# mpc001/auto_avsr

Hardware: AMD Instinct MI355X
Metric: video-frames/sec/node (25fps 88x88, max-frames=1600), E2E training step (fwd+bwd+clip+AdamW) (higher is better)
Workload: dtype f16 activations x f16x2 weights (atrunk3, atrunk4, decoder, encoder, trunk3, trunk4) + split-bf16 (everything else) forward / bf16 backward

## Files before the change

auto_avsr_amd/csrc/prims.h:

```cpp
#pragma once

extern "C" void avsr_note_launch(int err);
extern "C" int avsr_take_launch_error(void);
#ifdef AVSR_EMU
#include "hip_emu.h"
#define AVSR_LAUNCH(kern, grid, block, smem, stream, ...) \
    emu::launch((grid), (block), (smem), [=]() { kern(__VA_ARGS__); })
#define AVSR_DYN_SMEM(name) char* name = emu::dyn_smem()
#else
#include <hip/hip_runtime.h>
#define AVSR_LAUNCH(kern, grid, block, smem, stream, ...)                          \
    do {                                                                           \
        (void)hipGetLastError();                                                   \
        hipLaunchKernelGGL(kern, (grid), (block), (smem), (stream), __VA_ARGS__);  \
        avsr_note_launch((int)hipGetLastError());                                  \
    } while (0)
#define AVSR_DYN_SMEM(name) extern __shared__ __attribute__((aligned(16))) char name[]
#endif

#include <stdint.h>

#define AVSR_DEV __device__ __forceinline__
#define AVSR_WAVE 64

typedef uint16_t bf16_t;
typedef short bf16x8 __attribute__((ext_vector_type(8)));
typedef short bf16x4 __attribute__((ext_vector_type(4)));
typedef float f32x4 __attribute__((ext_vector_type(4)));
typedef float f32x16 __attribute__((ext_vector_type(16)));

AVSR_DEV float bf2f(bf16_t h) {
    uint32_t u = ((uint32_t)h) << 16;
    return __builtin_bit_cast(float, u);
}
AVSR_DEV bf16_t f2bf(float f) {
#ifndef AVSR_EMU
    return __builtin_bit_cast(bf16_t, (__bf16)f);
#endif
    uint32_t u = __builtin_bit_cast(uint32_t, f);
    if ((u & 0x7fffffffu) > 0x7f800000u) return (bf16_t)((u >> 16) | 0x40);
    u += 0x7fffu + ((u >> 16) & 1u);
    return (bf16_t)(u >> 16);
}

typedef _Float16 f16_t;
typedef _Float16 f16x8 __attribute__((ext_vector_type(8)));
typedef _Float16 f16x4 __attribute__((ext_vector_type(4)));
AVSR_DEV float h2f(f16_t h) { return (float)h; }
AVSR_DEV f16_t f2h(float f) {
#ifdef AVSR_EMU
    f = f > 65504.f ? 65504.f : (f < -65504.f ? -65504.f : f);
#else
    f = __builtin_amdgcn_fmed3f(f, -65504.f, 65504.f);
#endif
    return (f16_t)f;
}
AVSR_DEV short f2h_bits(float f) { return __builtin_bit_cast(short, f2h(f)); }
#define AVSR_H16_LO_SCALE 2048.0f
AVSR_DEV f16_t f2h_lo(float w) { return f2h((w - h2f(f2h(w))) * AVSR_H16_LO_SCALE); }

template <class T> struct Elem;
template <> struct Elem<float> {
    static AVSR_DEV float ld(const float* p) { return *p; }
    static AVSR_DEV void st(float* p, float v) { *p = v; }
};
template <> struct Elem<bf16_t> {
    static AVSR_DEV float ld(const bf16_t* p) { return bf2f(*p); }
    static AVSR_DEV void st(bf16_t* p, float v) { *p = f2bf(v); }
};
template <> struct Elem<f16_t> {
    static AVSR_DEV float ld(const f16_t* p) { return h2f(*p); }
    static AVSR_DEV void st(f16_t* p, float v) { *p = f2h(v); }
};

AVSR_DEV void load8(const bf16_t* p, float* out) {
    bf16x8 v = *reinterpret_cast<const bf16x8*>(p);
#pragma unroll
    for (int i = 0; i < 8; i++) out[i] = bf2f((bf16_t)v[i]);
}
AVSR_DEV void load8(const f16_t* p, float* out) {
    f16x8 v = *reinterpret_cast<const f16x8*>(p);
#pragma unroll
    for (int i = 0; i < 8; i++) out[i] = (float)v[i];
}
AVSR_DEV void load8(const float* p, float* out) {
    f32x4 a = *reinterpret_cast<const f32x4*>(p);
    f32x4 b = *reinterpret_cast<const f32x4*>(p + 4);
#pragma unroll
    for (int i = 0; i < 4; i++) {
        out[i] = a[i];
        out[i + 4] = b[i];
    }
}
AVSR_DEV void store8(bf16_t* p, const float* v) {
    bf16x8 o;
#pragma unroll
    for (int i = 0; i < 8; i++) o[i] = (short)f2bf(v[i]);
    *reinterpret_cast<bf16x8*>(p) = o;
}
AVSR_DEV void store8(f16_t* p, const float* v) {
    f16x8 o;
#pragma unroll
    for (int i = 0; i < 8; i++) o[i] = f2h(v[i]);
    *reinterpret_cast<f16x8*>(p) = o;
}
AVSR_DEV void store8_lo(f16_t* p, const float* v) {
    float l[8];
#pragma unroll
    for (int i = 0; i < 8; i++) l[i] = (v[i] - h2f(f2h(v[i]))) * AVSR_H16_LO_SCALE;
    store8(p, l);
}
AVSR_DEV void store8(float* p, const float* v) {
    f32x4 a, b;
#pragma unroll
    for (int i = 0; i < 4; i++) {
        a[i] = v[i];
        b[i] = v[i + 4];
    }
    *reinterpret_cast<f32x4*>(p) = a;
    *reinterpret_cast<f32x4*>(p + 4) = b;
}

AVSR_DEV void glds16(const void* gptr, void* lds_wave_base) {
#ifdef AVSR_EMU
    memcpy(reinterpret_cast<char*>(lds_wave_base) + 16 * emu::lane_id(), gptr, 16);
#else
    __builtin_amdgcn_global_load_lds((const __attribute__((address_space(1))) void*)gptr,
                                     (__attribute__((address_space(3))) void*)lds_wave_base, 16, 0, 0);
#endif
}
AVSR_DEV void block_barrier_raw() {
#ifdef AVSR_EMU
    emu::sync_threads();
#else
    __builtin_amdgcn_s_barrier();
#endif
}
AVSR_DEV int wave_id() {
#ifdef AVSR_EMU
    return (int)(threadIdx.x >> 6);
#else
    return __builtin_amdgcn_readfirstlane((int)(threadIdx.x >> 6));
#endif
}
AVSR_DEV void sched_fence() {
#ifndef AVSR_EMU
    __builtin_amdgcn_sched_barrier(0);
#endif
}
template <int N> AVSR_DEV void wait_vmcnt() {
#ifndef AVSR_EMU
    asm volatile("s_waitcnt vmcnt(%0)" ::"n"(N) : "memory");
#endif
}

AVSR_DEV bf16x4 lds_tr16(const bf16_t* p) {
#ifdef AVSR_EMU
    bf16x4 mine = *reinterpret_cast<const bf16x4*>(p);
    size_t stride;
    const unsigned char* all = emu::wave_gather(&mine, sizeof(mine), &stride);
    const int l = emu::lane_id(), i = l & 15, g = l >> 4;
    bf16x4 out;
    for (int j = 0; j < 4; j++) {
        bf16x4 src;
        memcpy(&src, all + (size_t)(16 * g + 4 * j + (i >> 2)) * stride, sizeof(src));
        out[j] = src[i & 3];
    }
    return out;
#else
    return __builtin_amdgcn_ds_read_tr16_b64_v4i16((__attribute__((address_space(3))) bf16x4*)p);
#endif
}

AVSR_DEV bf16x4 lds_tr16_async(const bf16_t* p) {
#ifdef AVSR_EMU
    return lds_tr16(p);
#else
    const uint32_t addr = (uint32_t)(uintptr_t)(const __attribute__((address_space(3))) bf16_t*)p;
    bf16x4 v;
    asm volatile("ds_read_b64_tr_b16 %0, %1" : "=v"(v) : "v"(addr));
    return v;
#endif
}
typedef int i32x4 __attribute__((ext_vector_type(4)));
typedef int i32x2 __attribute__((ext_vector_type(2)));
AVSR_DEV i32x4 lds_read16_async(const void* p) {
#ifdef AVSR_EMU
    i32x4 v;
    memcpy(&v, p, 16);
    return v;
#else
    const uint32_t addr = (uint32_t)(uintptr_t)(const __attribute__((address_space(3))) char*)p;
    i32x4 v;
    asm volatile("ds_read_b128 %0, %1" : "=v"(v) : "v"(addr));
    return v;
#endif
}
AVSR_DEV i32x2 lds_read8_async(const void* p) {
#ifdef AVSR_EMU
    i32x2 v;
    memcpy(&v, p, 8);
    return v;
#else
    const uint32_t addr = (uint32_t)(uintptr_t)(const __attribute__((address_space(3))) char*)p;
    i32x2 v;
    asm volatile("ds_read_b64 %0, %1" : "=v"(v) : "v"(addr));
    return v;
#endif
}
template <int N> AVSR_DEV void lds_wait() {
#ifndef AVSR_EMU
    asm volatile("s_waitcnt lgkmcnt(%0)" ::"n"(N));
#endif
}
template <class T> AVSR_DEV void lds_tie(T& v) {
#ifndef AVSR_EMU
    asm volatile("" : "+v"(v));
#endif
}

AVSR_DEV float avsr_exp(float x) {
#ifdef AVSR_EMU
    return expf(x);
#else
    return __expf(x);
#endif
}
AVSR_DEV float avsr_sigmoid(float x) {
#ifdef AVSR_EMU
    return 1.0f / (1.0f + avsr_exp(-x));
#else
    return __builtin_amdgcn_rcpf(1.0f + avsr_exp(-x));
#endif
}
AVSR_DEV float avsr_silu(float x) { return x * avsr_sigmoid(x); }

AVSR_DEV float wave_up1(float x, float fill) {
#ifdef AVSR_EMU
    const float v = __shfl_up(x, 1);
    return emu::lane_id() == 0 ? fill : v;
#else
    return __int_as_float(__builtin_amdgcn_update_dpp(__float_as_int(fill), __float_as_int(x), 0x138, 0xf, 0xf, false));
#endif
}
AVSR_DEV float wave_down1(float x, float fill) {
#ifdef AVSR_EMU
    const float v = __shfl_down(x, 1);
    return emu::lane_id() == 63 ? fill : v;
#else
    return __int_as_float(__builtin_amdgcn_update_dpp(__float_as_int(fill), __float_as_int(x), 0x130, 0xf, 0xf, false));
#endif
}

AVSR_DEV float wave_sum(float v) {
#pragma unroll
    for (int m = 32; m >= 1; m >>= 1) v += __shfl_xor(v, m);
    return v;
}
AVSR_DEV float wave_max(float v) {
#pragma unroll
    for (int m = 32; m >= 1; m >>= 1) v = fmaxf(v, __shfl_xor(v, m));
    return v;
}

AVSR_DEV f32x16 mfma32(bf16x8 a, bf16x8 b, f32x16 c) {
#ifdef AVSR_EMU
    struct P { bf16x8 a, b; } mine{a, b};
    size_t stride;
    const unsigned char* all = emu::wave_gather(&mine, sizeof(P), &stride);
    const int l = emu::lane_id();
    const int j = l & 31;
    for (int r = 0; r < 16; r++) {
        const int i = (r & 3) + 8 * (r >> 2) + 4 * (l >> 5);
        float acc = c[r];
        for (int kb = 0; kb < 2; kb++) {
            P pa, pb;
            memcpy(&pa, all + (size_t)(i + 32 * kb) * stride, sizeof(P));
            memcpy(&pb, all + (size_t)(j + 32 * kb) * stride, sizeof(P));
            for (int e = 0; e < 8; e++) acc += bf2f((bf16_t)pa.a[e]) * bf2f((bf16_t)pb.b[e]);
        }
        c[r] = acc;
    }
    return c;
#else
    typedef __bf16 v8bf __attribute__((ext_vector_type(8)));
    return __builtin_amdgcn_mfma_f32_32x32x16_bf16(__builtin_bit_cast(v8bf, a),
                                                   __builtin_bit_cast(v8bf, b), c, 0, 0, 0);
#endif
}
AVSR_DEV f32x16 mfma32_vgpr(bf16x8 a, bf16x8 b, f32x16 c) {
#ifdef AVSR_EMU
    return mfma32(a, b, c);
#else
    asm volatile("v_mfma_f32_32x32x16_bf16 %0, %1, %2, %0" : "+v"(c) : "v"(a), "v"(b));
    return c;
#endif
}
AVSR_DEV f32x4 mfma16(bf16x8 a, bf16x8 b, f32x4 c) {
#ifdef AVSR_EMU
    struct P { bf16x8 a, b; } mine{a, b};
    size_t stride;
    const unsigned char* all = emu::wave_gather(&mine, sizeof(P), &stride);
    const int l = emu::lane_id();
    const int j = l & 15;
    for (int r = 0; r < 4; r++) {
        const int i = 4 * (l >> 4) + r;
        float acc = c[r];
        for (int kb = 0; kb < 4; kb++) {
            P pa, pb;
            memcpy(&pa, all + (size_t)(i + 16 * kb) * stride, sizeof(P));
            memcpy(&pb, all + (size_t)(j + 16 * kb) * stride, sizeof(P));
            for (int e = 0; e < 8; e++) acc += bf2f((bf16_t)pa.a[e]) * bf2f((bf16_t)pb.b[e]);
        }
        c[r] = acc;
    }
    return c;
#else
    typedef __bf16 v8bf __attribute__((ext_vector_type(8)));
    return __builtin_amdgcn_mfma_f32_16x16x32_bf16(__builtin_bit_cast(v8bf, a),
                                                   __builtin_bit_cast(v8bf, b), c, 0, 0, 0);
#endif
}

template <int FMT> AVSR_DEV float raw16_to_f32(short bits) {
    return FMT == 1 ? (float)__builtin_bit_cast(f16_t, bits) : bf2f((bf16_t)bits);
}
template <int FMT> AVSR_DEV short f32_to_raw16(float v) { return FMT == 1 ? f2h_bits(v) : (short)f2bf(v); }
template <int FMT> AVSR_DEV f32x16 mfma32x(bf16x8 a, bf16x8 b, f32x16 c) {
    if (FMT == 0) return mfma32(a, b, c);
#ifdef AVSR_EMU
    struct P { bf16x8 a, b; } mine{a, b};
    size_t stride;
    const unsigned char* all = emu::wave_gather(&mine, sizeof(P), &stride);
    const int l = emu::lane_id();
    const int j = l & 31;
    for (int r = 0; r < 16; r++) {
        const int i = (r & 3) + 8 * (r >> 2) + 4 * (l >> 5);
        float acc = c[r];
        for (int kb = 0; kb < 2; kb++) {
            P pa, pb;
            memcpy(&pa, all + (size_t)(i + 32 * kb) * stride, sizeof(P));
            memcpy(&pb, all + (size_t)(j + 32 * kb) * stride, sizeof(P));
            for (int e = 0; e < 8; e++) acc += raw16_to_f32<1>(pa.a[e]) * raw16_to_f32<1>(pb.b[e]);
        }
        c[r] = acc;
    }
    return c;
#else
    return __builtin_amdgcn_mfma_f32_32x32x16_f16(__builtin_bit_cast(f16x8, a), __builtin_bit_cast(f16x8, b), c, 0, 0, 0);
#endif
}
template <int FMT> AVSR_DEV f32x4 mfma16x(bf16x8 a, bf16x8 b, f32x4 c) {
    if (FMT == 0) return mfma16(a, b, c);
#ifdef AVSR_EMU
    struct P { bf16x8 a, b; } mine{a, b};
    size_t stride;
    const unsigned char* all = emu::wave_gather(&mine, sizeof(P), &stride);
    const int l = emu::lane_id();
    const int j = l & 15;
    for (int r = 0; r < 4; r++) {
        const int i = 4 * (l >> 4) + r;
        float acc = c[r];
        for (int kb = 0; kb < 4; kb++) {
            P pa, pb;
            memcpy(&pa, all + (size_t)(i + 16 * kb) * stride, sizeof(P));
            memcpy(&pb, all + (size_t)(j + 16 * kb) * stride, sizeof(P));
            for (int e = 0; e < 8; e++) acc += raw16_to_f32<1>(pa.a[e]) * raw16_to_f32<1>(pb.b[e]);
        }
        c[r] = acc;
    }
    return c;
#else
    return __builtin_amdgcn_mfma_f32_16x16x32_f16(__builtin_bit_cast(f16x8, a), __builtin_bit_cast(f16x8, b), c, 0, 0, 0);
#endif
}

template <int NS> struct Frag { bf16x8 p[NS]; };

template <int NS>
AVSR_DEV f32x16 mma32(const Frag<NS>& a, const Frag<NS>& b, f32x16 c) {
    if (NS == 2) {
        c = mfma32(a.p[NS - 1], b.p[0], c);
        c = mfma32(a.p[0], b.p[NS - 1], c);
    }
    return mfma32(a.p[0], b.p[0], c);
}
template <int NS>
AVSR_DEV f32x4 mma16(const Frag<NS>& a, const Frag<NS>& b, f32x4 c) {
    if (NS == 2) {
        c = mfma16(a.p[NS - 1], b.p[0], c);
        c = mfma16(a.p[0], b.p[NS - 1], c);
    }
    return mfma16(a.p[0], b.p[0], c);
}

template <int NS> AVSR_DEV void split_bf16(float x, bf16_t* out) {
    bf16_t h = f2bf(x);
    out[0] = h;
    if (NS == 2) out[NS - 1] = f2bf(x - bf2f(h));
}

struct sp8_t { float raw; };
AVSR_DEV void load8(const sp8_t* p, float* out) {
    const bf16x8 hi = *reinterpret_cast<const bf16x8*>(p);
    const bf16x8 lo = *(reinterpret_cast<const bf16x8*>(p) + 1);
#pragma unroll
    for (int i = 0; i < 8; i++) out[i] = bf2f((bf16_t)hi[i]) + bf2f((bf16_t)lo[i]);
}
AVSR_DEV void store8(sp8_t* p, const float* v) {
    bf16x8 hi, lo;
#pragma unroll
    for (int i = 0; i < 8; i++) {
        bf16_t pl[2];
        split_bf16<2>(v[i], pl);
        hi[i] = (short)pl[0];
        lo[i] = (short)pl[1];
    }
    *reinterpret_cast<bf16x8*>(p) = hi;
    *(reinterpret_cast<bf16x8*>(p) + 1) = lo;
}
template <> struct Elem<sp8_t> {
    static AVSR_DEV float ld(const sp8_t*) { return 0.f; }
    static AVSR_DEV void st(sp8_t*, float) {}
};

AVSR_DEV uint32_t avsr_hash_key(uint64_t seed) {
    uint64_t z = seed + 0x9E3779B97F4A7C15ull;
    z = (z ^ (z >> 30)) * 0xBF58476D1CE4E5B9ull;
    z = (z ^ (z >> 27)) * 0x94D049BB133111EBull;
    z = z ^ (z >> 31);
    return (uint32_t)(z >> 32);
}
AVSR_DEV uint32_t avsr_mix32(uint32_t x) {
    x ^= x >> 16;
    x *= 0x7feb352du;
    x ^= x >> 15;
    x *= 0x846ca68bu;
    x ^= x >> 16;
    return x;
}
AVSR_DEV uint32_t avsr_hash(uint64_t seed, uint64_t idx) {
    uint32_t x = avsr_mix32((uint32_t)idx ^ avsr_hash_key(seed));
    const uint32_t hi = (uint32_t)(idx >> 32);
    if (hi) x = avsr_mix32(x + hi * 0x9E3779B1u);
    return x;
}
AVSR_DEV float dropout_scale(uint64_t seed, uint64_t idx, float p, float inv_keep) {
    if (p <= 0.f) return 1.f;
    const float u = (float)(avsr_hash(seed, idx) >> 8) * (1.0f / 16777216.0f);
    return u < p ? 0.f : inv_keep;
}

extern int avsr_tune_knobs[32];
inline bool avsr_det() { return avsr_tune_knobs[23] != 0; }
int avsr_colsum_det(const void* src, int dtype, long ld, long rows, int cols, float* out, hipStream_t stream);
int avsr_rowsum_det_bf16(const void* src, long ld, long rows, long cols, float* out, hipStream_t stream);
extern "C" void avsr_set_error(const char* msg);
extern "C" void avsr_set_error2(const char* where, const char* what);
#define AVSR_CHECK_LAUNCH(name)                                                   \
    do {                                                                          \
        int e__ = avsr_take_launch_error();                                       \
        if (e__ != 0) {                                                           \
            avsr_set_error2(name, hipGetErrorString((hipError_t)e__));            \
            return 2;                                                             \
        }                                                                         \
    } while (0)
#define AVSR_REQUIRE(cond, msg)         \
    do {                                \
        if (!(cond)) {                  \
            avsr_set_error(msg);        \
            return 1;                   \
        }                               \
    } while (0)
```

auto_avsr_amd/csrc/stem.hip:

```cpp
#include "prims.h"
#include "avsr_hip.h"

namespace {

constexpr int KT = 5, KH = 7, KW = 7, ROWS = KT * KH;
constexpr int KP = 288;
constexpr int CO = 64;
constexpr int LP = 104;

template <int NS>
__global__ void stem_weight_kernel(const float* __restrict__ w, bf16_t* __restrict__ wp) {
    const int i = blockIdx.x * 256 + threadIdx.x;
    if (i >= CO * KP) return;
    const int co = i / KP, k = i % KP, r = k >> 3, j = k & 7;
    bf16_t pl[NS];
    split_bf16<NS>((r < ROWS && j >= 1) ? w[(co * ROWS + r) * KW + j - 1] : 0.f, pl);
#pragma unroll
    for (int q = 0; q < NS; q++) wp[q * CO * KP + i] = pl[q];
}

constexpr int PATCH_V = 4;
template <int NS = 1>
AVSR_DEV void patch_init(bf16_t* patch, int W) {
    for (int i = threadIdx.x; i < 36 * LP; i += 256) {
        const int r = i / LP, c = i - r * LP;
        if (r == 35 || c < 4 || c >= 4 + W)
#pragma unroll
            for (int q = 0; q < NS; q++) patch[q * 36 * LP + i] = 0;
    }
}
AVSR_DEV void patch_load(f32x4 (&q)[PATCH_V], const float* __restrict__ x, long row, int OH, int T, int H, int W) {
    const int n = (int)(row / OH), oh = (int)(row - (long)n * OH);
    const int b = n / T, t = n - b * T;
    const int nv = W >> 2;
#pragma unroll
    for (int j = 0; j < PATCH_V; j++) {
        const int i = threadIdx.x + 256 * j;
        q[j] = f32x4{0.f, 0.f, 0.f, 0.f};
        if (i < ROWS * nv) {
            const int r = i / nv, v = i - r * nv;
            const int kt = r / KH, kh = r - kt * KH;
            const int tt = t + kt - 2, ih = 2 * oh + kh - 3;
            if (tt >= 0 && tt < T && ih >= 0 && ih < H)
                q[j] = *reinterpret_cast<const f32x4*>(x + (((long)b * T + tt) * H + ih) * W + v * 4);
        }
    }
}
template <int NS = 1>
AVSR_DEV void patch_store(bf16_t* patch, const f32x4 (&q)[PATCH_V], int W) {
    const int nv = W >> 2;
#pragma unroll
    for (int j = 0; j < PATCH_V; j++) {
        const int i = threadIdx.x + 256 * j;
        if (i < ROWS * nv) {
            const int r = i / nv, v = i - r * nv;
            bf16x4 o[NS];
#pragma unroll
            for (int e = 0; e < 4; e++) {
                bf16_t pl[NS];
                split_bf16<NS>(q[j][e], pl);
#pragma unroll
                for (int s = 0; s < NS; s++) o[s][e] = (short)pl[s];
            }
#pragma unroll
            for (int s = 0; s < NS; s++)
                *reinterpret_cast<bf16x4*>(patch + s * 36 * LP + r * LP + 4 + v * 4) = o[s];
        }
    }
}

AVSR_DEV bf16x8 patch_frag(const bf16_t* patch, int r, int ow) {
    const uint32_t* p = reinterpret_cast<const uint32_t*>(patch + r * LP + 2 * ow);
    bf16x8 f;
#pragma unroll
    for (int e = 0; e < 4; e++) {
        const uint32_t u = p[e];
        f[2 * e] = (short)(u & 0xffff);
        f[2 * e + 1] = (short)(u >> 16);
    }
    return f;
}

constexpr int FWD_ROWS = 8;
constexpr int OP = 72;

template <int NS, class TO>
__global__ __launch_bounds__(256) void stem_fwd_kernel(const float* __restrict__ x, const bf16_t* __restrict__ wp,
                                                       TO* __restrict__ y, int T, int H, int W, int OH, int OW,
                                                       long total_rows, bf16_t* __restrict__ y2 = nullptr,
                                                       float* __restrict__ stats_part = nullptr) {
    constexpr int OPT = sizeof(TO) == 2 ? OP : 68;
    __shared__ __attribute__((aligned(16))) bf16_t patch[NS * 36 * LP];
    __shared__ __attribute__((aligned(16))) TO orow[64 * OPT];
    const int lane = threadIdx.x & 63, w = threadIdx.x >> 6;
    const int quad = lane >> 4, lc = lane & 15;
    Frag<NS> fb[9];
#pragma unroll
    for (int ks = 0; ks < 9; ks++)
#pragma unroll
        for (int q = 0; q < NS; q++)
            fb[ks].p[q] = *reinterpret_cast<const bf16x8*>(wp + q * CO * KP + (16 * w + lc) * KP + ks * 32 + 8 * quad);
    const int ntile = (OW + 15) / 16;
    const long row_end = min(total_rows, ((long)blockIdx.x + 1) * FWD_ROWS);
    patch_init<NS>(patch, W);
    f32x4 q[PATCH_V];
    patch_load(q, x, (long)blockIdx.x * FWD_ROWS, OH, T, H, W);
    f32x4 st1 = f32x4{0.f, 0.f, 0.f, 0.f}, st2 = f32x4{0.f, 0.f, 0.f, 0.f};
    for (long row = (long)blockIdx.x * FWD_ROWS; row < row_end; row++) {
        __syncthreads();
        patch_store<NS>(patch, q, W);
        if (row + 1 < row_end) patch_load(q, x, row + 1, OH, T, H, W);
        __syncthreads();
        for (int mt = 0; mt < ntile; mt++) {
            const int ow = min(mt * 16 + lc, OW - 1);
            f32x4 acc = f32x4{0.f, 0.f, 0.f, 0.f};
#pragma unroll
            for (int ks = 0; ks < 9; ks++) {
                Frag<NS> fx;
#pragma unroll
                for (int s = 0; s < NS; s++) fx.p[s] = patch_frag(patch + s * 36 * LP, ks * 4 + quad, ow);
                acc = mma16<NS>(fb[ks], fx, acc);
            }
            TO* o = orow + (mt * 16 + lc) * OPT + 16 * w + 4 * quad;
            if (sizeof(TO) == 2) {
                *reinterpret_cast<bf16x4*>(o) = bf16x4{(short)f2bf(acc[0]), (short)f2bf(acc[1]), (short)f2bf(acc[2]), (short)f2bf(acc[3])};
            } else {
                *reinterpret_cast<f32x4*>(o) = acc;
            }
        }
        __syncthreads();
        TO* dst = y + (row * OW) * CO;
        constexpr int EPC = 16 / sizeof(TO), CPP = CO / EPC;
        for (int i = threadIdx.x; i < OW * CPP; i += 256) {
            const int pix = i / CPP, c = (i % CPP) * EPC;
            const f32x4 v = *reinterpret_cast<const f32x4*>(orow + pix * OPT + c);
            *reinterpret_cast<f32x4*>(dst + pix * CO + c) = v;
            if (sizeof(TO) == 4 && stats_part) {
#pragma unroll
                for (int e = 0; e < 4; e++) {
                    st1[e] += v[e];
                    st2[e] += v[e] * v[e];
                }
            }
            if (sizeof(TO) == 4 && y2)
                *reinterpret_cast<bf16x4*>(y2 + (row * OW + pix) * CO + c) =
                    bf16x4{(short)f2bf(v[0]), (short)f2bf(v[1]), (short)f2bf(v[2]), (short)f2bf(v[3])};
        }
    }
    if (sizeof(TO) == 4 && stats_part) {
        __syncthreads();
        float* red = reinterpret_cast<float*>(orow);
        const int grp = threadIdx.x >> 4, c = (threadIdx.x & 15) * 4;
#pragma unroll
        for (int e = 0; e < 4; e++) {
            red[(grp * 2 + 0) * CO + c + e] = st1[e];
            red[(grp * 2 + 1) * CO + c + e] = st2[e];
        }
        __syncthreads();
        if (threadIdx.x < 2 * CO) {
            float v = 0.f;
#pragma unroll
            for (int g2 = 0; g2 < 16; g2++) v += red[g2 * 2 * CO + threadIdx.x];
            stats_part[(size_t)blockIdx.x * 2 * CO + threadIdx.x] = v;
        }
    }
}

constexpr int EP = 56;
constexpr int EO_ARR = 36 * EP;
constexpr int DYP = 64;

AVSR_DEV void eo_load(float (&v)[28], const float* __restrict__ x, long row, int OH, int T, int H, int W) {
    const int tid = threadIdx.x;
    if (tid >= ROWS * 6) return;
    const int n = (int)(row / OH), oh = (int)(row - (long)n * OH);
    const int b = n / T, t = n - b * T;
    const int r = tid / 6, g = tid - r * 6;
    const int kt = r / KH, kh = r - kt * KH;
    const int tt = t + kt - 2, ih = 2 * oh + kh - 3;
    const bool row_ok = tt >= 0 && tt < T && ih >= 0 && ih < H;
    const float* src = x + (((long)b * T + tt) * H + ih) * W;
#pragma unroll
    for (int q = 0; q < 7; q++) {
        const int c = 16 * g - 4 + 4 * q;
        f32x4 f = f32x4{0.f, 0.f, 0.f, 0.f};
        if (row_ok && c >= 0 && c + 3 < W) f = *reinterpret_cast<const f32x4*>(src + c);
        else if (row_ok)
#pragma unroll
            for (int e = 0; e < 4; e++) f[e] = (c + e >= 0 && c + e < W) ? src[c + e] : 0.f;
#pragma unroll
        for (int e = 0; e < 4; e++) v[4 * q + e] = f[e];
    }
}
AVSR_DEV void eo_store(bf16_t* eo, const float (&v)[28]) {
    const int tid = threadIdx.x;
    if (tid >= ROWS * 6) return;
    const int r = tid / 6, g = tid - r * 6;
#pragma unroll
    for (int par = 0; par < 2; par++)
#pragma unroll
        for (int sh = 0; sh < 4; sh++) {
            bf16x8 o;
#pragma unroll
            for (int m = 0; m < 8; m++) o[m] = (short)f2bf(v[1 + 2 * (m + sh) + par]);
            *reinterpret_cast<bf16x8*>(eo + (par * 4 + sh) * EO_ARR + r * EP + 8 * g) = o;
        }
}

__global__ __launch_bounds__(256) void stem_wgrad_kernel(const bf16_t* __restrict__ dy, const float* __restrict__ x,
                                                         float* __restrict__ partial, int T, int H, int W, int OH, int OW,
                                                         long total_rows) {
    __shared__ __attribute__((aligned(16))) bf16_t eo[8 * EO_ARR];
    __shared__ __attribute__((aligned(16))) bf16_t dyt[64 * DYP];
    const int lane = threadIdx.x & 63, w = threadIdx.x >> 6;
    const int quad = lane >> 4, lc = lane & 15;
    f32x4 acc[5][4];
#pragma unroll
    for (int j = 0; j < 5; j++)
#pragma unroll
        for (int m = 0; m < 4; m++) acc[j][m] = f32x4{0.f, 0.f, 0.f, 0.f};
    for (int i = threadIdx.x; i < 64 * DYP / 8; i += 256) reinterpret_cast<bf16x8*>(dyt)[i] = bf16x8{0, 0, 0, 0, 0, 0, 0, 0};
    for (int i = threadIdx.x; i < 8 * EP / 8; i += 256) {
        const int arr = i / (EP / 8), c8 = (i - arr * (EP / 8)) * 8;
        *reinterpret_cast<bf16x8*>(eo + arr * EO_ARR + 35 * EP + c8) = bf16x8{0, 0, 0, 0, 0, 0, 0, 0};
    }
    for (int i = threadIdx.x; i < 8 * 36; i += 256)
        *reinterpret_cast<bf16x8*>(eo + (i / 36) * EO_ARR + (i % 36) * EP + 48) = bf16x8{0, 0, 0, 0, 0, 0, 0, 0};
    int a_off[5];
#pragma unroll
    for (int j = 0; j < 5; j++) {
        const int kq = 16 * min(w + 4 * j, 17) + lc, r = kq >> 3, kw = kq & 7;
        a_off[j] = ((kw & 1) * 4 + (kw >> 1)) * EO_ARR + r * EP + 8 * quad;
    }
    const int b_row = 8 * quad + (lc >> 2), b_col = 4 * (lc & 3);
    float xv[28];
    bf16x8 dv[2];
    auto dy_load = [&](long row) {
#pragma unroll
        for (int j = 0; j < 2; j++) {
            const int i = threadIdx.x + 256 * j;
            dv[j] = bf16x8{0, 0, 0, 0, 0, 0, 0, 0};
            if (i < OW * 8) dv[j] = *reinterpret_cast<const bf16x8*>(dy + (row * OW + (i >> 3)) * CO + (i & 7) * 8);
        }
    };
    if ((long)blockIdx.x < total_rows) {
        eo_load(xv, x, blockIdx.x, OH, T, H, W);
        dy_load(blockIdx.x);
    }
    for (long row = blockIdx.x; row < total_rows; row += gridDim.x) {
        __syncthreads();
        eo_store(eo, xv);
#pragma unroll
        for (int j = 0; j < 2; j++) {
            const int i = threadIdx.x + 256 * j;
            if (i < OW * 8) *reinterpret_cast<bf16x8*>(dyt + (i >> 3) * DYP + (i & 7) * 8) = dv[j];
        }
        if (row + gridDim.x < total_rows) {
            eo_load(xv, x, row + gridDim.x, OH, T, H, W);
            dy_load(row + gridDim.x);
        }
        __syncthreads();
#pragma unroll
        for (int ks = 0; ks < 2; ks++) {
            bf16x8 fbm[4];
#pragma unroll
            for (int m = 0; m < 4; m++) {
                const bf16_t* p0 = dyt + (ks * 32 + b_row) * DYP + 16 * m + b_col;
                const bf16x4 lo = lds_tr16(p0), hi = lds_tr16(p0 + 4 * DYP);
                fbm[m] = bf16x8{lo[0], lo[1], lo[2], lo[3], hi[0], hi[1], hi[2], hi[3]};
            }
#pragma unroll
            for (int j = 0; j < 5; j++) {
                if (w + 4 * j >= 18) continue;
                const bf16x8 fa = *reinterpret_cast<const bf16x8*>(eo + a_off[j] + ks * 32);
#pragma unroll
                for (int m = 0; m < 4; m++) acc[j][m] = mfma16(fa, fbm[m], acc[j][m]);
            }
        }
    }
    float* out = partial + (long)blockIdx.x * KP * CO;
#pragma unroll
    for (int j = 0; j < 5; j++) {
        const int nt = w + 4 * j;
        if (nt >= 18) continue;
#pragma unroll
        for (int m = 0; m < 4; m++)
#pragma unroll
            for (int r = 0; r < 4; r++) out[(16 * nt + 4 * quad + r) * CO + 16 * m + lc] = acc[j][m][r];
    }
}

__global__ __launch_bounds__(1024) void stem_wgrad_reduce_kernel(const float* __restrict__ partial, int G,
                                                                 float* __restrict__ dw) {
    __shared__ float part[16][64];
    const int tx = threadIdx.x & 63, tz = threadIdx.x >> 6;
    const int i = blockIdx.x * 64 + tx;
    float s = 0.f;
    if (i < KP * CO)
        for (int g = tz; g < G; g += 16) s += partial[(long)g * KP * CO + i];
    part[tz][tx] = s;
    __syncthreads();
    if (tz != 0 || i >= KP * CO) return;
#pragma unroll
    for (int q = 1; q < 16; q++) s += part[q][tx];
    const int kq = i / CO, co = i - kq * CO, r = kq >> 3, kw = kq & 7;
    if (r < ROWS && kw < KW) dw[(co * ROWS + r) * KW + kw] = s;
}

}

constexpr int WG_MAX = 1024;
extern "C" int64_t avsr_stem357_workspace_bytes(void) { return (int64_t)WG_MAX * KP * CO * 4 + (int64_t)2 * CO * KP * 2; }

extern "C" int avsr_stem357_fwd(const float* x, const float* w, void* y, void* workspace, int B, int T, int H, int W,
                                hipStream_t stream) {
    AVSR_REQUIRE(W % 4 == 0 && W <= 96 && H >= 1, "stem357: W must be a multiple of 4 and <= 96");
    static_assert(ROWS * 24 <= PATCH_V * 256, "patch prefetch registers");
    if (B <= 0 || T <= 0) return 0;
    const int OH = (H + 6 - KH) / 2 + 1, OW = (W + 6 - KW) / 2 + 1;
    bf16_t* wp = reinterpret_cast<bf16_t*>(reinterpret_cast<char*>(workspace) + (size_t)WG_MAX * KP * CO * 4);
    AVSR_LAUNCH(stem_weight_kernel<1>, dim3((CO * KP + 255) / 256), dim3(256), 0, stream, w, wp);
    const long rows = (long)B * T * OH;
    AVSR_REQUIRE(OW <= 64, "stem357: at most 64 output columns");
    AVSR_LAUNCH((stem_fwd_kernel<1, bf16_t>), dim3((unsigned)((rows + FWD_ROWS - 1) / FWD_ROWS)), dim3(256), 0, stream, x,
                (const bf16_t*)wp, (bf16_t*)y, T, H, W, OH, OW, rows);
    AVSR_CHECK_LAUNCH("stem357_fwd");
    return 0;
}

static int stem357_fwd_f32s_impl(const float* x, const float* w, float* y, void* y2, void* workspace, int B, int T, int H, int W,
                                 float* stats_part, int stats_rows, hipStream_t stream) {
    AVSR_REQUIRE(W % 4 == 0 && W <= 96 && H >= 1, "stem357: W must be a multiple of 4 and <= 96");
    if (B <= 0 || T <= 0) return 0;
    const int OH = (H + 6 - KH) / 2 + 1, OW = (W + 6 - KW) / 2 + 1;
    bf16_t* wp = reinterpret_cast<bf16_t*>(reinterpret_cast<char*>(workspace) + (size_t)WG_MAX * KP * CO * 4);
    AVSR_LAUNCH(stem_weight_kernel<2>, dim3((CO * KP + 255) / 256), dim3(256), 0, stream, w, wp);
    const long rows = (long)B * T * OH;
    AVSR_REQUIRE(OW <= 64, "stem357: at most 64 output columns");
    const long blocks = (rows + FWD_ROWS - 1) / FWD_ROWS;
    AVSR_REQUIRE(stats_part == nullptr || stats_rows >= blocks, "stem357: statistics buffer too small");
    AVSR_LAUNCH((stem_fwd_kernel<2, float>), dim3((unsigned)blocks), dim3(256), 0, stream, x, (const bf16_t*)wp, y, T, H, W, OH, OW, rows,
                (bf16_t*)y2, stats_part);
    AVSR_CHECK_LAUNCH("stem357_fwd_f32s");
    return 0;
}

extern "C" int avsr_stem357_fwd_f32s(const float* x, const float* w, float* y, void* y2, void* workspace, int B, int T, int H,
                                     int W, hipStream_t stream) {
    return stem357_fwd_f32s_impl(x, w, y, y2, workspace, B, T, H, W, nullptr, 0, stream);
}
extern "C" int64_t avsr_stem357_stat_rows(int B, int T, int H) {
    const int OH = (H + 6 - KH) / 2 + 1;
    return ((int64_t)B * T * OH + FWD_ROWS - 1) / FWD_ROWS;
}
extern "C" int avsr_stem357_fwd_f32s_stats(const float* x, const float* w, float* y, void* y2, void* workspace, int B, int T, int H,
                                           int W, float* stats_part, int stats_rows, hipStream_t stream) {
    AVSR_REQUIRE(stats_part != nullptr, "stem357_fwd_f32s_stats: statistics buffer required");
    return stem357_fwd_f32s_impl(x, w, y, y2, workspace, B, T, H, W, stats_part, stats_rows, stream);
}

extern "C" int avsr_stem357_wgrad(const void* dy, const float* x, float* dw, void* workspace, int B, int T, int H, int W,
                                  hipStream_t stream) {
    AVSR_REQUIRE(W % 4 == 0 && W <= 96, "stem357: W must be a multiple of 4 and <= 96");
    if (B <= 0 || T <= 0) return 0;
    const int OH = (H + 6 - KH) / 2 + 1, OW = (W + 6 - KW) / 2 + 1;
    AVSR_REQUIRE(OW <= 64, "stem357: at most 64 output columns");
    const long rows = (long)B * T * OH;
    int gmax = avsr_tune_knobs[6] > 0 ? avsr_tune_knobs[6] : 512;
    if (gmax > WG_MAX) gmax = WG_MAX;
    const int G = (int)(rows < gmax ? rows : gmax);
    float* partial = reinterpret_cast<float*>(workspace);
    AVSR_LAUNCH(stem_wgrad_kernel, dim3(G), dim3(256), 0, stream, (const bf16_t*)dy, x, partial, T, H, W, OH, OW, rows);
    AVSR_LAUNCH(stem_wgrad_reduce_kernel, dim3((KP * CO + 63) / 64), dim3(1024), 0, stream, (const float*)partial, G, dw);
    AVSR_CHECK_LAUNCH("stem357_wgrad");
    return 0;
}
```

Before: 70110.

## Add row-group stem forward and weight-grad kernels with XCD-aware persistent scheduling

Adds new stem 3D conv forward and weight-gradient kernels that handle groups of 4 output rows per iteration. Each persistent block walks a contiguous range of groups, remapped so neighbouring ranges share an XCD, and prefetches the next group's input and dy into registers while computing the current one. The aim is to reuse the overlapping input rows across neighbouring output rows and to hide global load latency. Both kernels become the default, and the old per-row path stays behind a tune knob. The new weight-grad path also caps output width at 48 columns.

Result: faster. 70880 (median of 6 runs) (+1.1%).

```diff
diff --git a/auto_avsr_amd/csrc/prims.h b/auto_avsr_amd/csrc/prims.h
--- a/auto_avsr_amd/csrc/prims.h
+++ b/auto_avsr_amd/csrc/prims.h
@@ -146,6 +146,11 @@
 AVSR_DEV void sched_fence() {
 #ifndef AVSR_EMU
     __builtin_amdgcn_sched_barrier(0);
+#endif
+}
+template <class T> AVSR_DEV void reg_opaque(T& v) {
+#ifndef AVSR_EMU
+    asm volatile("" : "+v"(v));
 #endif
 }
 template <int N> AVSR_DEV void wait_vmcnt() {
diff --git a/auto_avsr_amd/csrc/stem.hip b/auto_avsr_amd/csrc/stem.hip
--- a/auto_avsr_amd/csrc/stem.hip
+++ b/auto_avsr_amd/csrc/stem.hip
@@ -290,6 +290,341 @@
     }
 }
 
+constexpr int WG_R = 4;
+constexpr int WG_PX = 48;
+constexpr int WG_IR = 2 * WG_R + 5;
+constexpr int WG_XR = KT * WG_IR;
+constexpr int WG_ARR = WG_XR * EP;
+constexpr int WG_XG = 7;
+constexpr int WG_XT = 2;
+constexpr int WG_DT = WG_R * WG_PX * 8 / 256;
+
+struct WgGroup {
+    int b, t, oh0;
+    long row0;
+};
+AVSR_DEV WgGroup wg_group(long grp, int GPF, int T, int OH) {
+    const int n = (int)(grp / GPF), gi = (int)(grp - (long)n * GPF);
+    WgGroup g;
+    g.b = n / T;
+    g.t = n - g.b * T;
+    g.oh0 = gi * WG_R;
+    g.row0 = (long)n * OH + g.oh0;
+    return g;
+}
+AVSR_DEV int xcd_block() {
+    const int b = blockIdx.x, total = gridDim.x, xcd = b & 7, slot = b >> 3, q = total >> 3, r = total & 7;
+    return (xcd < r ? xcd * (q + 1) : r * (q + 1) + (xcd - r) * q) + slot;
+}
+AVSR_DEV void rr_x_load(float (&v)[WG_XT][20], const float* __restrict__ x, const WgGroup& gp, int T, int H, int W) {
+#pragma unroll
+    for (int jt = 0; jt < WG_XT; jt++) {
+        const int i = min((int)threadIdx.x + 256 * jt, WG_XR * WG_XG - 1);
+        const int rs = i / WG_XG, g = i - rs * WG_XG;
+        const int kt = rs / WG_IR, li = rs - kt * WG_IR;
+        const int tt = min(max(gp.t + kt - 2, 0), T - 1), ih = min(max(2 * gp.oh0 - 3 + li, 0), H - 1);
+        const float* src = x + (((long)gp.b * T + tt) * H + ih) * W;
+#pragma unroll
+        for (int q = 0; q < 5; q++) {
+            const int c = min(max(16 * g - 4 + 4 * q, 0), W - 4);
+            const f32x4 f = *reinterpret_cast<const f32x4*>(src + c);
+#pragma unroll
+            for (int e = 0; e < 4; e++) v[jt][4 * q + e] = f[e];
+        }
+    }
+}
+AVSR_DEV void rr_x_store(bf16_t* eo, const float (&v)[WG_XT][20], const WgGroup& gp, int T, int H, int W) {
+#pragma unroll
+    for (int jt = 0; jt < WG_XT; jt++) {
+        const int i = threadIdx.x + 256 * jt;
+        if (i >= WG_XR * WG_XG) continue;
+        const int rs = i / WG_XG, g = i - rs * WG_XG;
+        const int kt = rs / WG_IR, li = rs - kt * WG_IR;
+        const int tt = gp.t + kt - 2, ih = 2 * gp.oh0 - 3 + li;
+        const bool row_ok = tt >= 0 && tt < T && ih >= 0 && ih < H;
+        bf16_t c[19];
+#pragma unroll
+        for (int j = 0; j < 19; j++) {
+            const int col = 16 * g - 4 + ((1 + j) & ~3);
+            c[j] = (row_ok && col >= 0 && col < W) ? f2bf(v[jt][1 + j]) : (bf16_t)0;
+        }
+#pragma unroll
+        for (int par = 0; par < 2; par++)
+#pragma unroll
+            for (int sh = 0; sh < 2; sh++) {
+                bf16x8 o;
+#pragma unroll
+                for (int m = 0; m < 8; m++) o[m] = (short)c[2 * (m + sh) + par];
+                *reinterpret_cast<bf16x8*>(eo + (par * 2 + sh) * WG_ARR + rs * EP + 8 * g) = o;
+            }
+    }
+}
+
+__global__ __launch_bounds__(256, 2) void stem_wgrad_rr_kernel(const bf16_t* __restrict__ dy, const float* __restrict__ x,
+                                                               float* __restrict__ partial, int T, int H, int W, int OH, int OW,
+                                                               int GPF, long groups, int per_block) {
+    __shared__ __attribute__((aligned(16))) bf16_t eo[4 * WG_ARR];
+    __shared__ __attribute__((aligned(16))) bf16_t dyt[WG_R * WG_PX * DYP];
+    const int lane = threadIdx.x & 63, w = wave_id();
+    const int quad = lane >> 4, lc = lane & 15;
+    const int lb = xcd_block();
+    const long g_begin = (long)lb * per_block, g_end = min(groups, g_begin + per_block);
+    f32x4 acc[5][4];
+#pragma unroll
+    for (int j = 0; j < 5; j++)
+#pragma unroll
+        for (int m = 0; m < 4; m++) acc[j][m] = f32x4{0.f, 0.f, 0.f, 0.f};
+    for (int i = threadIdx.x; i < WG_R * WG_PX * DYP / 8; i += 256) reinterpret_cast<bf16x8*>(dyt)[i] = bf16x8{0, 0, 0, 0, 0, 0, 0, 0};
+    int a_off[5];
+#pragma unroll
+    for (int j = 0; j < 5; j++) {
+        const int kq = 16 * min(w + 4 * j, 17) + lc, r = min(kq >> 3, ROWS - 1), kw = kq & 7;
+        const int kt = r / KH, kh = r - kt * KH;
+        a_off[j] = ((kw & 1) * 2 + ((kw >> 1) & 1)) * WG_ARR + (kt * WG_IR + kh) * EP + 2 * (kw >> 2);
+    }
+    int k_off[6];
+#pragma unroll
+    for (int ks = 0; ks < 6; ks++) {
+        const int s = 4 * ks + quad, jr = s / 6;
+        k_off[ks] = 2 * jr * EP + 8 * (s - 6 * jr);
+    }
+    const int b_row = 8 * quad + (lc >> 2), b_col = 4 * (lc & 3);
+    float xv[WG_XT][20];
+    bf16x8 dv[WG_DT];
+    auto dy_load = [&](const WgGroup& gp) {
+#pragma unroll
+        for (int jt = 0; jt < WG_DT; jt++) {
+            const int i = threadIdx.x + 256 * jt;
+            const int j = i / (WG_PX * 8), rem = i - j * (WG_PX * 8), pix = rem >> 3;
+            dv[jt] = *reinterpret_cast<const bf16x8*>(dy + ((gp.row0 + min(j, OH - 1 - gp.oh0)) * OW + min(pix, OW - 1)) * CO + (rem & 7) * 8);
+        }
+    };
+    if (g_begin < g_end) {
+        const WgGroup gp = wg_group(g_begin, GPF, T, OH);
+        rr_x_load(xv, x, gp, T, H, W);
+        dy_load(gp);
+    }
+    for (long grp = g_begin; grp < g_end; grp++) {
+        __syncthreads();
+        const WgGroup cur = wg_group(grp, GPF, T, OH);
+        const int cur_oh0 = cur.oh0;
+        rr_x_store(eo, xv, cur, T, H, W);
+#pragma unroll
+        for (int jt = 0; jt < WG_DT; jt++) {
+            const int i = threadIdx.x + 256 * jt;
+            const bool row_ok = cur_oh0 + i / (WG_PX * 8) < OH;
+            if (((i % (WG_PX * 8)) >> 3) < OW)
+                *reinterpret_cast<bf16x8*>(dyt + (i >> 3) * DYP + (i & 7) * 8) = row_ok ? dv[jt] : bf16x8{0, 0, 0, 0, 0, 0, 0, 0};
+        }
+        if (grp + 1 < g_end) {
+            const WgGroup gp = wg_group(grp + 1, GPF, T, OH);
+            rr_x_load(xv, x, gp, T, H, W);
+            dy_load(gp);
+        }
+        __syncthreads();
+#pragma unroll
+        for (int ks = 0; ks < 6; ks++) {
+            bf16x8 fbm[4];
+#pragma unroll
+            for (int m = 0; m < 4; m++) {
+                const bf16_t* p0 = dyt + (ks * 32 + b_row) * DYP + 16 * m + b_col;
+                const bf16x4 lo = lds_tr16(p0), hi = lds_tr16(p0 + 4 * DYP);
+                fbm[m] = bf16x8{lo[0], lo[1], lo[2], lo[3], hi[0], hi[1], hi[2], hi[3]};
+            }
+            auto a_frag = [&](int j) {
+                const uint32_t* p = reinterpret_cast<const uint32_t*>(eo + a_off[j] + k_off[ks]);
+                bf16x8 f;
+#pragma unroll
+                for (int e = 0; e < 4; e++) {
+                    const uint32_t u = p[e];
+                    f[2 * e] = (short)(u & 0xffff);
+                    f[2 * e + 1] = (short)(u >> 16);
+                }
+                return f;
+            };
+            bf16x8 fa = a_frag(0);
+#pragma unroll
+            for (int j = 0; j < 5; j++) {
+                if (j == 4 && w >= 2) continue;
+                bf16x8 fn = fa;
+                if (j < 3 || (j == 3 && w < 2)) fn = a_frag(j + 1);
+#pragma unroll
+                for (int m = 0; m < 4; m++) acc[j][m] = mfma16(fa, fbm[m], acc[j][m]);
+                fa = fn;
+            }
+        }
+    }
+    float* out = partial + (long)lb * KP * CO;
+#pragma unroll
+    for (int j = 0; j < 5; j++) {
+        const int nt = w + 4 * j;
+        if (nt >= 18) continue;
+#pragma unroll
+        for (int m = 0; m < 4; m++)
+#pragma unroll
+            for (int r = 0; r < 4; r++) out[(16 * nt + 4 * quad + r) * CO + 16 * m + lc] = acc[j][m][r];
+    }
+}
+
+constexpr int FG_R = WG_R;
+constexpr int FG_IR = 2 * FG_R + 5, FG_XR = KT * FG_IR;
+constexpr int FG_ROWS = FG_XR + 2 * (FG_R - 1) + 1;
+constexpr int FG_V = 7;
+constexpr int FG_GRID = 512;
+static_assert(FG_XR * 24 <= FG_V * 256, "patch prefetch registers");
+
+template <int NS>
+AVSR_DEV void rg_patch_init(bf16_t* patch, int W) {
+    for (int i = threadIdx.x; i < FG_ROWS * LP; i += 256) {
+        const int r = i / LP, c = i - r * LP;
+        if (r >= FG_XR || c < 4 || c >= 4 + W)
+#pragma unroll
+            for (int q = 0; q < NS; q++) patch[q * FG_ROWS * LP + i] = 0;
+    }
+}
+AVSR_DEV void rg_patch_load(f32x4 (&q)[FG_V], const float* __restrict__ x, const WgGroup& gp, int T, int H, int W) {
+    const int nv = W >> 2, inv = (65536 + nv - 1) / nv;
+#pragma unroll
+    for (int j = 0; j < FG_V; j++) {
+        int i = min((int)threadIdx.x + 256 * j, FG_XR * nv - 1);
+        reg_opaque(i);
+        const int rs = (i * inv) >> 16, v = i - rs * nv;
+        const int kt = rs / FG_IR, li = rs - kt * FG_IR;
+        const int tt = min(max(gp.t + kt - 2, 0), T - 1), ih = min(max(2 * gp.oh0 - 3 + li, 0), H - 1);
+        q[j] = *reinterpret_cast<const f32x4*>(x + (((long)gp.b * T + tt) * H + ih) * W + v * 4);
+    }
+}
+template <int NS>
+AVSR_DEV void rg_patch_store(bf16_t* patch, const f32x4 (&q)[FG_V], const WgGroup& gp, int T, int H, int W) {
+    const int nv = W >> 2, inv = (65536 + nv - 1) / nv;
+#pragma unroll
+    for (int j = 0; j < FG_V; j++) {
+        int i = threadIdx.x + 256 * j;
+        reg_opaque(i);
+        if (i < FG_XR * nv) {
+            const int rs = (i * inv) >> 16, v = i - rs * nv;
+            const int kt = rs / FG_IR, li = rs - kt * FG_IR;
+            const int tt = gp.t + kt - 2, ih = 2 * gp.oh0 - 3 + li;
+            const bool ok = tt >= 0 && tt < T && ih >= 0 && ih < H;
+            bf16x4 o[NS];
+#pragma unroll
+            for (int e = 0; e < 4; e++) {
+                bf16_t pl[NS];
+                split_bf16<NS>(ok ? q[j][e] : 0.f, pl);
+#pragma unroll
+                for (int s = 0; s < NS; s++) o[s][e] = (short)pl[s];
+            }
+#pragma unroll
+            for (int s = 0; s < NS; s++) *reinterpret_cast<bf16x4*>(patch + s * FG_ROWS * LP + rs * LP + 4 + v * 4) = o[s];
+        }
+    }
+}
+
+template <int NS, class TO>
+__global__ __launch_bounds__(256, 2) void stem_fwd_rg_kernel(const float* __restrict__ x, const bf16_t* __restrict__ wp,
+                                                             TO* __restrict__ y, int T, int H, int W, int OH, int OW, int GPF,
+                                                             long groups, int per_block, bf16_t* __restrict__ y2,
+                                                             float* __restrict__ stats_part) {
+    constexpr int PL = FG_ROWS * LP;
+    __shared__ __attribute__((aligned(16))) bf16_t patch[NS * PL];
+    __shared__ float red[2][2 * CO];
+    const int lane = threadIdx.x & 63, w = wave_id();
+    const int quad = lane >> 4, lc = lane & 15;
+    const int ch = w & 1, ph = w >> 1;
+    Frag<NS> fb[2][9];
+#pragma unroll
+    for (int g = 0; g < 2; g++)
+#pragma unroll
+        for (int ks = 0; ks < 9; ks++)
+#pragma unroll
+            for (int q = 0; q < NS; q++)
+                fb[g][ks].p[q] = *reinterpret_cast<const bf16x8*>(wp + q * CO * KP + (32 * ch + 16 * g + lc) * KP + ks * 32 + 8 * quad);
+    int roff[9];
+#pragma unroll
+    for (int ks = 0; ks < 9; ks++) {
+        const int r = 4 * ks + quad, kt = r / KH;
+        roff[ks] = (r < ROWS ? kt * FG_IR + (r - kt * KH) : FG_XR) * LP;
+    }
+    const int lb = xcd_block();
+    const long g_begin = (long)lb * per_block, g_end = min(groups, g_begin + per_block);
+    const int npix = FG_R * OW, ntile = (npix + 15) >> 4;
+    rg_patch_init<NS>(patch, W);
+    f32x4 q[FG_V];
+    if (g_begin < g_end) rg_patch_load(q, x, wg_group(g_begin, GPF, T, OH), T, H, W);
+    f32x4 st1[2], st2[2];
+#pragma unroll
+    for (int g = 0; g < 2; g++) st1[g] = st2[g] = f32x4{0.f, 0.f, 0.f, 0.f};
+    for (long grp = g_begin; grp < g_end; grp++) {
+        const WgGroup gp = wg_group(grp, GPF, T, OH);
+        __syncthreads();
+        rg_patch_store<NS>(patch, q, gp, T, H, W);
+        if (grp + 1 < g_end) rg_patch_load(q, x, wg_group(grp + 1, GPF, T, OH), T, H, W);
+        __syncthreads();
+        const int nvalid = min(FG_R, OH - gp.oh0) * OW;
+        const long pix0 = gp.row0 * OW;
+        for (int t = ph; t < ntile; t += 2) {
+            const int p = 16 * t + lc, pc = min(p, npix - 1);
+            const int j = pc / OW, ow = pc - j * OW;
+            const bf16_t* base = patch + 2 * j * LP + 2 * ow;
+            f32x4 a0 = f32x4{0.f, 0.f, 0.f, 0.f}, a1 = a0;
+#pragma unroll
+            for (int ks = 0; ks < 9; ks++) {
+                Frag<NS> fx;
+#pragma unroll
+                for (int s = 0; s < NS; s++) fx.p[s] = patch_frag(base + s * PL + roff[ks], 0, 0);
+                if (NS == 2) {
+                    a0 = mfma16(fb[0][ks].p[NS - 1], fx.p[0], a0);
+                    a1 = mfma16(fb[1][ks].p[NS - 1], fx.p[0], a1);
+                    a0 = mfma16(fb[0][ks].p[0], fx.p[NS - 1], a0);
+                    a1 = mfma16(fb[1][ks].p[0], fx.p[NS - 1], a1);
+                }
+                a0 = mfma16(fb[0][ks].p[0], fx.p[0], a0);
+                a1 = mfma16(fb[1][ks].p[0], fx.p[0], a1);
+            }
+            if (p < nvalid) {
+                const long o = (pix0 + p) * CO + 32 * ch + 4 * quad;
+#pragma unroll
+                for (int g = 0; g < 2; g++) {
+                    const f32x4 v = g ? a1 : a0;
+                    const bf16x4 vb = bf16x4{(short)f2bf(v[0]), (short)f2bf(v[1]), (short)f2bf(v[2]), (short)f2bf(v[3])};
+                    if (sizeof(TO) == 2) {
+                        *reinterpret_cast<bf16x4*>(y + o + 16 * g) = vb;
+                    } else {
+                        *reinterpret_cast<f32x4*>(y + o + 16 * g) = v;
+                        if (y2) *reinterpret_cast<bf16x4*>(y2 + o + 16 * g) = vb;
+                        if (stats_part) {
+#pragma unroll
+                            for (int e = 0; e < 4; e++) {
+                                st1[g][e] += v[e];
+                                st2[g][e] += v[e] * v[e];
+                            }
+                        }
+                    }
+                }
+            }
+        }
+    }
+    if (sizeof(TO) == 4 && stats_part) {
+#pragma unroll
+        for (int g = 0; g < 2; g++)
+#pragma unroll
+            for (int e = 0; e < 4; e++) {
+                float v1 = st1[g][e], v2 = st2[g][e];
+#pragma unroll
+                for (int m = 1; m < 16; m <<= 1) {
+                    v1 += __shfl_xor(v1, m);
+                    v2 += __shfl_xor(v2, m);
+                }
+                if (lc == 0) {
+                    red[ph][32 * ch + 16 * g + 4 * quad + e] = v1;
+                    red[ph][CO + 32 * ch + 16 * g + 4 * quad + e] = v2;
+                }
+            }
+        __syncthreads();
+        if (threadIdx.x < 2 * CO) stats_part[(size_t)blockIdx.x * 2 * CO + threadIdx.x] = red[0][threadIdx.x] + red[1][threadIdx.x];
+    }
+}
+
 __global__ __launch_bounds__(1024) void stem_wgrad_reduce_kernel(const float* __restrict__ partial, int G,
                                                                  float* __restrict__ dw) {
     __shared__ float part[16][64];
@@ -309,12 +644,25 @@
 
 }
 
+struct FwdGrid {
+    int gpf, per_block;
+    long groups, blocks;
+};
+static FwdGrid fwd_grid(int B, int T, int OH) {
+    FwdGrid g;
+    g.gpf = (OH + FG_R - 1) / FG_R;
+    g.groups = (long)B * T * g.gpf;
+    g.per_block = (int)((g.groups + FG_GRID - 1) / FG_GRID);
+    g.blocks = (g.groups + g.per_block - 1) / g.per_block;
+    return g;
+}
+
 constexpr int WG_MAX = 1024;
 extern "C" int64_t avsr_stem357_workspace_bytes(void) { return (int64_t)WG_MAX * KP * CO * 4 + (int64_t)2 * CO * KP * 2; }
 
 extern "C" int avsr_stem357_fwd(const float* x, const float* w, void* y, void* workspace, int B, int T, int H, int W,
                                 hipStream_t stream) {
-    AVSR_REQUIRE(W % 4 == 0 && W <= 96 && H >= 1, "stem357: W must be a multiple of 4 and <= 96");
+    AVSR_REQUIRE(W % 4 == 0 && W >= 4 && W <= 96 && H >= 1, "stem357: W must be a multiple of 4 in 4 .. 96");
     static_assert(ROWS * 24 <= PATCH_V * 256, "patch prefetch registers");
     if (B <= 0 || T <= 0) return 0;
     const int OH = (H + 6 - KH) / 2 + 1, OW = (W + 6 - KW) / 2 + 1;
@@ -322,25 +670,37 @@
     AVSR_LAUNCH(stem_weight_kernel<1>, dim3((CO * KP + 255) / 256), dim3(256), 0, stream, w, wp);
     const long rows = (long)B * T * OH;
     AVSR_REQUIRE(OW <= 64, "stem357: at most 64 output columns");
-    AVSR_LAUNCH((stem_fwd_kernel<1, bf16_t>), dim3((unsigned)((rows + FWD_ROWS - 1) / FWD_ROWS)), dim3(256), 0, stream, x,
-                (const bf16_t*)wp, (bf16_t*)y, T, H, W, OH, OW, rows);
+    if (avsr_tune_knobs[28] == 1) {
+        AVSR_LAUNCH((stem_fwd_kernel<1, bf16_t>), dim3((unsigned)((rows + FWD_ROWS - 1) / FWD_ROWS)), dim3(256), 0, stream, x,
+                    (const bf16_t*)wp, (bf16_t*)y, T, H, W, OH, OW, rows);
+    } else {
+        const FwdGrid fg = fwd_grid(B, T, OH);
+        AVSR_LAUNCH((stem_fwd_rg_kernel<1, bf16_t>), dim3((unsigned)fg.blocks), dim3(256), 0, stream, x, (const bf16_t*)wp, (bf16_t*)y, T, H,
+                    W, OH, OW, fg.gpf, fg.groups, fg.per_block, (bf16_t*)nullptr, (float*)nullptr);
+    }
     AVSR_CHECK_LAUNCH("stem357_fwd");
     return 0;
 }
 
 static int stem357_fwd_f32s_impl(const float* x, const float* w, float* y, void* y2, void* workspace, int B, int T, int H, int W,
                                  float* stats_part, int stats_rows, hipStream_t stream) {
-    AVSR_REQUIRE(W % 4 == 0 && W <= 96 && H >= 1, "stem357: W must be a multiple of 4 and <= 96");
+    AVSR_REQUIRE(W % 4 == 0 && W >= 4 && W <= 96 && H >= 1, "stem357: W must be a multiple of 4 in 4 .. 96");
     if (B <= 0 || T <= 0) return 0;
     const int OH = (H + 6 - KH) / 2 + 1, OW = (W + 6 - KW) / 2 + 1;
     bf16_t* wp = reinterpret_cast<bf16_t*>(reinterpret_cast<char*>(workspace) + (size_t)WG_MAX * KP * CO * 4);
     AVSR_LAUNCH(stem_weight_kernel<2>, dim3((CO * KP + 255) / 256), dim3(256), 0, stream, w, wp);
     const long rows = (long)B * T * OH;
     AVSR_REQUIRE(OW <= 64, "stem357: at most 64 output columns");
-    const long blocks = (rows + FWD_ROWS - 1) / FWD_ROWS;
+    const FwdGrid fg = fwd_grid(B, T, OH);
+    const bool per_row = avsr_tune_knobs[28] == 1;
+    const long blocks = per_row ? (rows + FWD_ROWS - 1) / FWD_ROWS : fg.blocks;
     AVSR_REQUIRE(stats_part == nullptr || stats_rows >= blocks, "stem357: statistics buffer too small");
-    AVSR_LAUNCH((stem_fwd_kernel<2, float>), dim3((unsigned)blocks), dim3(256), 0, stream, x, (const bf16_t*)wp, y, T, H, W, OH, OW, rows,
-                (bf16_t*)y2, stats_part);
+    if (per_row)
+        AVSR_LAUNCH((stem_fwd_kernel<2, float>), dim3((unsigned)blocks), dim3(256), 0, stream, x, (const bf16_t*)wp, y, T, H, W, OH, OW, rows,
+                    (bf16_t*)y2, stats_part);
+    else
+        AVSR_LAUNCH((stem_fwd_rg_kernel<2, float>), dim3((unsigned)blocks), dim3(256), 0, stream, x, (const bf16_t*)wp, y, T, H, W, OH, OW,
+                    fg.gpf, fg.groups, fg.per_block, (bf16_t*)y2, stats_part);
     AVSR_CHECK_LAUNCH("stem357_fwd_f32s");
     return 0;
 }
@@ -351,7 +711,8 @@
 }
 extern "C" int64_t avsr_stem357_stat_rows(int B, int T, int H) {
     const int OH = (H + 6 - KH) / 2 + 1;
-    return ((int64_t)B * T * OH + FWD_ROWS - 1) / FWD_ROWS;
+    if (avsr_tune_knobs[28] == 1) return ((int64_t)B * T * OH + FWD_ROWS - 1) / FWD_ROWS;
+    return fwd_grid(B, T, OH).blocks;
 }
 extern "C" int avsr_stem357_fwd_f32s_stats(const float* x, const float* w, float* y, void* y2, void* workspace, int B, int T, int H,
                                            int W, float* stats_part, int stats_rows, hipStream_t stream) {
@@ -361,16 +722,27 @@
 
 extern "C" int avsr_stem357_wgrad(const void* dy, const float* x, float* dw, void* workspace, int B, int T, int H, int W,
                                   hipStream_t stream) {
-    AVSR_REQUIRE(W % 4 == 0 && W <= 96, "stem357: W must be a multiple of 4 and <= 96");
+    AVSR_REQUIRE(W % 4 == 0 && W >= 4 && W <= 96 && H >= 1, "stem357: W must be a multiple of 4 in 4 .. 96");
     if (B <= 0 || T <= 0) return 0;
     const int OH = (H + 6 - KH) / 2 + 1, OW = (W + 6 - KW) / 2 + 1;
     AVSR_REQUIRE(OW <= 64, "stem357: at most 64 output columns");
     const long rows = (long)B * T * OH;
     int gmax = avsr_tune_knobs[6] > 0 ? avsr_tune_knobs[6] : 512;
     if (gmax > WG_MAX) gmax = WG_MAX;
-    const int G = (int)(rows < gmax ? rows : gmax);
     float* partial = reinterpret_cast<float*>(workspace);
-    AVSR_LAUNCH(stem_wgrad_kernel, dim3(G), dim3(256), 0, stream, (const bf16_t*)dy, x, partial, T, H, W, OH, OW, rows);
+    int G;
+    if (avsr_tune_knobs[28] == 1) {
+        G = (int)(rows < gmax ? rows : gmax);
+        AVSR_LAUNCH(stem_wgrad_kernel, dim3(G), dim3(256), 0, stream, (const bf16_t*)dy, x, partial, T, H, W, OH, OW, rows);
+    } else {
+        AVSR_REQUIRE(OW <= WG_PX, "stem357: at most 48 output columns");
+        const int GPF = (OH + WG_R - 1) / WG_R;
+        const long groups = (long)B * T * GPF;
+        const long per_block = (groups + gmax - 1) / gmax;
+        G = (int)((groups + per_block - 1) / per_block);
+        AVSR_LAUNCH(stem_wgrad_rr_kernel, dim3(G), dim3(256), 0, stream, (const bf16_t*)dy, x, partial, T, H, W, OH, OW, GPF, groups,
+                    (int)per_block);
+    }
     AVSR_LAUNCH(stem_wgrad_reduce_kernel, dim3((KP * CO + 63) / 64), dim3(1024), 0, stream, (const float*)partial, G, dw);
     AVSR_CHECK_LAUNCH("stem357_wgrad");
     return 0;
```
